# s0phia-/tetris

Hardware: AMD Instinct MI355X
Metric: env-steps/sec (higher is better)
Workload: dtype u32; 1 GPU; 1048576 envs/GPU x 1 GPU, 10x20 board, pieces=default, uniform random valid actions, in-kernel auto-reset, device bag seed 0; envs_per_gpu=1048576, observation_output=True, env_steps_per_launch=1, steps_per_graph_replay=1, streams_per_gpu=1, board=10x20, pieces=default, backend=single, device=cuda

## Files before the change

### tetris_amd/csrc/tetris_core.hpp

```cpp
#pragma once
#include <stdint.h>

#if defined(__HIPCC__)
#include <hip/hip_runtime.h>
#define TET_HD __host__ __device__ __forceinline__
#else
#define TET_HD inline
#endif

#ifndef TET_ABLATE
#define TET_ABLATE 0
#endif
#ifndef TET_BAG_SMALL_PATH
#define TET_BAG_SMALL_PATH 1
#endif
#ifndef TET_RESCUE_SKIP
#define TET_RESCUE_SKIP 1
#endif

#ifndef TET_FENCE_EVERY
#define TET_FENCE_EVERY 2
#endif
#ifndef TET_FENCE_MASK
#define TET_FENCE_MASK 1
#endif
#if defined(__HIP_DEVICE_COMPILE__)
#define TET_SCHED_FENCE() __builtin_amdgcn_sched_barrier(0)
#define TET_PIN(x) asm volatile("" : "+v"(x))
#else
#define TET_SCHED_FENCE() ((void)0)
#define TET_PIN(x) ((void)0)
#endif

#if defined(__HIP_DEVICE_COMPILE__)
#define TET_WAVE_ANY(x) (__ballot((x)) != 0ull)
#else
#define TET_WAVE_ANY(x) (x)
#endif

#if defined(__HIP_DEVICE_COMPILE__)
#define TET_SCRATCH_OR(ptr, v) ((void)__hip_atomic_fetch_or((ptr), (v), __ATOMIC_RELAXED, __HIP_MEMORY_SCOPE_WORKGROUP))
#else
#define TET_SCRATCH_OR(ptr, v) (*(ptr) |= (v))
#endif

#if defined(__HIP_DEVICE_COMPILE__)
#define TET_FMUL(a, b) __fmul_rn((a), (b))
#define TET_FADD(a, b) __fadd_rn((a), (b))
#else
#define TET_FMUL(a, b) ((float)((volatile float)(a) * (b)))
#define TET_FADD(a, b) ((float)((volatile float)(a) + (b)))
#endif

namespace tet {

constexpr int kMaxPieces = 12;
constexpr int kMaxCols = 12;
constexpr int kNumCatalogue = 9;

struct Orient {
  int w, H, b[4], n[4];
  bool exists;
};

TET_HD Orient unpack_orient(uint32_t d) {
  Orient o;
  o.w = d & 7;
  o.H = (d >> 3) & 7;
#pragma unroll
  for (int j = 0; j < 4; ++j) {
    o.b[j] = (d >> (6 + 5 * j)) & 3;
    o.n[j] = (d >> (8 + 5 * j)) & 7;
  }
  o.exists = (d >> 31) != 0;
  return o;
}

#ifndef TET_NO_PACK
#define TET_NO_PACK 0
#endif
TET_HD constexpr bool board_packed(int word_bytes, int num_rows) { return !TET_NO_PACK && num_rows + 4 <= 6 * word_bytes; }
TET_HD constexpr int n_planes(int C, bool packed) { return packed ? (C / 4) * 3 + ((C % 4) * 3 + 3) / 4 : C; }
constexpr int kTileEnvs = 64;
TET_HD constexpr int64_t plane_index(int64_t i, int p, int NP) { return ((i >> 6) * NP + p) * kTileEnvs + (i & 63); }
TET_HD constexpr int64_t board_words(int64_t B, int NP) { return ((B + kTileEnvs - 1) / kTileEnvs) * NP * kTileEnvs; }

template <typename W, int C, bool PACK>
TET_HD void unpack_board(const W (&w)[n_planes(C, PACK)], W (&col)[C]) {
  if (!PACK) {
#pragma unroll
    for (int c = 0; c < C; ++c) col[c] = w[c < n_planes(C, PACK) ? c : 0];
    return;
  }
  constexpr int Wb = 8 * (int)sizeof(W), F = Wb * 3 / 4, P = n_planes(C, PACK);
  const W M = (W)(((W)1 << F) - 1);
#pragma unroll
  for (int g = 0; 4 * g < C; ++g) {
    const int b = 3 * g, c0 = 4 * g;
    const W w0 = w[b], w1 = w[b + 1 < P ? b + 1 : b], w2 = w[b + 2 < P ? b + 2 : b];
    col[c0] = (W)(w0 & M);
    if (c0 + 1 < C) col[c0 + 1] = (W)(((w0 >> F) | (w1 << (Wb - F))) & M);
    if (c0 + 2 < C) col[c0 + 2] = (W)(((w1 >> (2 * F - Wb)) | (w2 << (2 * Wb - 2 * F))) & M);
    if (c0 + 3 < C) col[c0 + 3] = (W)(w2 >> (3 * F - 2 * Wb));
  }
}

template <typename W, int C, bool PACK>
TET_HD void pack_board(const W (&col)[C], W (&w)[n_planes(C, PACK)]) {
  if (!PACK) {
#pragma unroll
    for (int c = 0; c < n_planes(C, PACK); ++c) w[c] = col[c < C ? c : 0];
    return;
  }
  constexpr int Wb = 8 * (int)sizeof(W), F = Wb * 3 / 4, P = n_planes(C, PACK);
#pragma unroll
  for (int g = 0; 4 * g < C; ++g) {
    const int b = 3 * g, c0 = 4 * g;
    const W x0 = col[c0], x1 = c0 + 1 < C ? col[c0 + 1 < C ? c0 + 1 : c0] : (W)0;
    const W x2 = c0 + 2 < C ? col[c0 + 2 < C ? c0 + 2 : c0] : (W)0, x3 = c0 + 3 < C ? col[c0 + 3 < C ? c0 + 3 : c0] : (W)0;
    w[b] = (W)(x0 | (x1 << F));
    if (b + 1 < P) w[b + 1 < P ? b + 1 : b] = (W)((x1 >> (Wb - F)) | (x2 << (2 * F - Wb)));
    if (b + 2 < P) w[b + 2 < P ? b + 2 : b] = (W)((x2 >> (2 * Wb - 2 * F)) | (x3 << (3 * F - 2 * Wb)));
  }
}

template <typename W, int C, bool PACK>
TET_HD void load_board(const W* planes, int64_t , int64_t i, W (&col)[C]) {
  constexpr int NP = n_planes(C, PACK);
  W w[NP];
  const W* rec = planes + plane_index(i, 0, NP);
#pragma unroll
  for (int p = 0; p < NP; ++p) w[p] = rec[p * kTileEnvs];
  unpack_board<W, C, PACK>(w, col);
}
template <typename W, int C, bool PACK>
TET_HD void store_board(W* planes, int64_t , int64_t i, const W (&col)[C]) {
  constexpr int NP = n_planes(C, PACK);
  W w[NP];
  pack_board<W, C, PACK>(col, w);
  W* rec = planes + plane_index(i, 0, NP);
#pragma unroll
  for (int p = 0; p < NP; ++p) rec[p * kTileEnvs] = w[p];
}

template <typename W>
TET_HD W load_column_rt(const W* planes, int64_t , int64_t i, int c, int C, bool packed) {
  const int NP = n_planes(C, packed);
  if (!packed) return planes[plane_index(i, c, NP)];
  constexpr int Wb = 8 * (int)sizeof(W), F = Wb * 3 / 4;
  const W M = (W)(((W)1 << F) - 1);
  const int b = 3 * (c >> 2), k = c & 3;
  const W lo = planes[plane_index(i, b + (k == 0 ? 0 : k - 1), NP)];
  if (k == 0) return (W)(lo & M);
  if (k == 3) return (W)(lo >> (3 * F - 2 * Wb));
  const W hi = planes[plane_index(i, b + k, NP)];
  return k == 1 ? (W)(((lo >> F) | (hi << (Wb - F))) & M) : (W)(((lo >> (2 * F - Wb)) | (hi << (2 * Wb - 2 * F))) & M);
}
template <typename W>
TET_HD void store_columns_rt(W* planes, int64_t , int64_t i, const W* col, int C, bool packed) {
  if (!packed) {
    for (int c = 0; c < C; ++c) planes[plane_index(i, c, C)] = col[c];
    return;
  }
  constexpr int Wb = 8 * (int)sizeof(W), F = Wb * 3 / 4;
  const int P = n_planes(C, true);
  for (int p = 0; p < P; ++p) {
    const int c0 = 4 * (p / 3), q = p % 3;
    const W a = c0 + q < C ? col[c0 + q] : (W)0, b = c0 + q + 1 < C ? col[c0 + q + 1] : (W)0;
    const W v = q == 0 ? (W)(a | (b << F))
                       : (q == 1 ? (W)((a >> (Wb - F)) | (b << (2 * F - Wb))) : (W)((a >> (2 * Wb - 2 * F)) | (b << (3 * F - 2 * Wb))));
    planes[plane_index(i, p, P)] = v;
  }
}

constexpr uint64_t kMaskBits = (1ull << 48) - 1;
constexpr int kFieldStride = 12;
TET_HD constexpr int mask_bit(int k, int c) { return kFieldStride * k + c; }
TET_HD uint64_t meta_pack(uint64_t mask, int piece, uint32_t bag) {
  return (mask & kMaskBits) | ((uint64_t)(piece & 15) << 48) | ((uint64_t)(bag & 0xFFF) << 52);
}
TET_HD uint64_t meta_mask(uint64_t m) { return m & kMaskBits; }
TET_HD int meta_piece(uint64_t m) { return (int)((m >> 48) & 15); }
TET_HD uint32_t meta_bag(uint64_t m) { return (uint32_t)(m >> 52); }

TET_HD int popc(uint32_t x) { return __builtin_popcount(x); }
TET_HD int popc(uint64_t x) { return __builtin_popcountll(x); }
TET_HD int bitlen(uint32_t x) { return 31 - __builtin_clz((x << 1) | 1u); }
TET_HD int bitlen(uint64_t x) { return 63 - __builtin_clzll((x << 1) | 1ull); }
TET_HD uint32_t umin(uint32_t a, uint32_t b) { return a < b ? a : b; }
TET_HD int nlz_above(uint32_t x) { return __builtin_clz((x << 1) | 1u); }
TET_HD int nlz_above(uint64_t x) { return __builtin_clzll((x << 1) | 1ull); }
template <typename W>
TET_HD W lowmask(int n) { return (W)(((W)1 << n) - 1); }

TET_HD uint32_t sad_u8(uint32_t a, uint32_t b, uint32_t acc) {
#if defined(__HIP_DEVICE_COMPILE__)
  return __builtin_amdgcn_sad_u8(a, b, acc);
#else
  for (int k = 0; k < 4; ++k) {
    const int d = (int)((a >> (8 * k)) & 255u) - (int)((b >> (8 * k)) & 255u);
    acc += (uint32_t)(d < 0 ? -d : d);
  }
  return acc;
#endif
}

TET_HD uint32_t mix32(uint32_t x) {
  x ^= x >> 16;
  x *= 0x7feb352dU;
  x ^= x >> 15;
  x *= 0x846ca68bU;
  x ^= x >> 16;
  return x;
}
TET_HD uint32_t hash_key(uint64_t seed, uint64_t counter) {
  uint32_t k = mix32((uint32_t)seed ^ 0x9E3779B9U);
  k = mix32(k ^ (uint32_t)(seed >> 32));
  k = mix32(k ^ (uint32_t)counter);
  k = mix32(k ^ (uint32_t)(counter >> 32));
  return k;
}
TET_HD uint32_t hash_env(uint32_t key, uint32_t env) {
  uint32_t h = (key ^ env) * 0x9E3779B1U;
  h ^= h >> 16;
  h *= 0x85EBCA6BU;
  h ^= h >> 13;
  return h;
}
TET_HD int scale16(uint32_t r16, int n) { return (int)((r16 * (uint32_t)n) >> 16); }

TET_HD int select_bit32(uint32_t v, int k) {
  int pos = 0;
  int c = popc(v & 0xFFFFu);
  if (k >= c) { k -= c; pos += 16; v >>= 16; }
  c = popc(v & 0xFFu);
  if (k >= c) { k -= c; pos += 8; v >>= 8; }
  c = popc(v & 0xFu);
  if (k >= c) { k -= c; pos += 4; v >>= 4; }
  c = popc(v & 0x3u);
  if (k >= c) { k -= c; pos += 2; v >>= 2; }
  c = (int)(v & 1u);
  if (k >= c) { pos += 1; }
  return pos;
}
TET_HD int bag_draw(uint32_t& bag, int n_pieces, uint32_t r16) {
  if (bag == 0) bag = (1u << n_pieces) - 1u;
  const int k = scale16(r16, popc(bag));
  uint32_t v = bag;
  int pos = 0;
  int c = popc(v & 0xFFu);
  if (k >= c) { pos = 8; v >>= 8; }
  int kk = k >= c ? k - c : k;
  c = popc(v & 0xFu);
  if (kk >= c) { kk -= c; pos += 4; v >>= 4; }
  c = popc(v & 0x3u);
  if (kk >= c) { kk -= c; pos += 2; v >>= 2; }
  c = (int)(v & 1u);
  if (kk >= c) pos += 1;
  bag &= ~(1u << pos);
  return pos;
}

TET_HD int bag_draw_lut(uint32_t& bag, int n_pieces, uint32_t r16, const uint8_t* sel_nib) {
  if (bag == 0) bag = (1u << n_pieces) - 1u;
#if TET_BAG_SMALL_PATH
  if (n_pieces <= 4) {
    const int k4 = scale16(r16, popc(bag));
    const int pos4 = (int)sel_nib[bag * 4u + (uint32_t)k4];
    bag &= ~(1u << pos4);
    return pos4;
  }
#endif
  int k = scale16(r16, popc(bag));
  const int c0 = popc(bag & 0xFu), c1 = c0 + popc(bag & 0xF0u);
  const int grp = (k >= c0) + (k >= c1);
  k -= grp == 0 ? 0 : (grp == 1 ? c0 : c1);
  const uint32_t nib = (bag >> (4 * grp)) & 15u;
  const int pos = 4 * grp + (int)sel_nib[nib * 4u + (uint32_t)k];
  bag &= ~(1u << pos);
  return pos;
}

struct alignas(16) OrientEntry {
  uint32_t sh[4];
  uint32_t rj0[2];
  uint32_t rj1[2];
  uint32_t vert4;
  uint32_t set_w4;
  uint32_t desc;
  uint32_t pad_;
};
static_assert(sizeof(OrientEntry) == 48, "table staging and LDS reads assume 48-byte entries");

struct alignas(16) StampRow {
  uint32_t shape4;
  uint32_t bias4;
  uint32_t H;
  uint32_t pad_;
};
constexpr uint32_t kNoColumn = 64;
static_assert(sizeof(StampRow) == 16, "one ds_read_b128");

struct SetTable {
  OrientEntry orient[kMaxPieces][4];
  uint64_t fullmask[kMaxPieces];
  StampRow stamp[kMaxPieces][4];
};

TET_HD const OrientEntry* piece_entries(const SetTable& tab, int np) {
  uint32_t off = (uint32_t)np * (uint32_t)sizeof(tab.orient[0]);
  TET_PIN(off);
  return reinterpret_cast<const OrientEntry*>(reinterpret_cast<const char*>(&tab.orient[0][0]) + off);
}

template <int CR>
struct LutLayout {
  static constexpr int kHoleEntries = 1 << (CR + 1), kWellsEntries = 1 << CR;
  static constexpr int kHoleA = 0, kHoleU = kHoleEntries, kWellsS = 2 * kHoleEntries;
  static constexpr int kWellsLead = kWellsS + kWellsEntries, kWellsTrail = kWellsLead + kWellsEntries;
  static constexpr int kSelPair = kWellsTrail + kWellsEntries, kSelNib = kSelPair + 256 * 8;
  static constexpr int kByteTablesEnd = kSelNib + 16 * 4;
  static constexpr int kPackHole = kByteTablesEnd, kPackWells = kPackHole + 2 * kHoleEntries;
  static constexpr int kBytes = CR == 10 ? kPackWells + 4 * kWellsEntries : kByteTablesEnd;
};
template <typename W, int C, int NCH, int CR, bool PACKW = false>
TET_HD constexpr bool features_packed() { return sizeof(W) == 4 && C <= 10 && NCH == 2 && CR == 10 && !PACKW; }
constexpr int kFeatureLutBytes = LutLayout<12>::kBytes;
constexpr int kFeatureLut10Bytes = LutLayout<10>::kBytes;
struct AfterLut {
  static constexpr int kHoleA = LutLayout<12>::kHoleA, kHoleU = LutLayout<12>::kHoleU;
  static constexpr int kWellsPack = 2 * LutLayout<12>::kHoleEntries;
  static constexpr int kSelPair = kWellsPack + 4 * LutLayout<12>::kWellsEntries, kSelNib = kSelPair + 256 * 8;
  static constexpr int kBytes = kSelNib + 16 * 4;
};
constexpr int kAfterLutBytes = AfterLut::kBytes;

TET_HD uint32_t spread2(uint32_t x) {
  x = (x | (x << 8)) & 0x00FF00FFu;
  x = (x | (x << 4)) & 0x0F0F0F0Fu;
  x = (x | (x << 2)) & 0x33333333u;
  x = (x | (x << 1)) & 0x55555555u;
  return x;
}

template <int C>
TET_HD uint32_t mask_field(uint64_t mask, int k) { return (uint32_t)(mask >> (kFieldStride * k)) & ((1u << C) - 1u); }

template <int C>
TET_HD void slot_of_action_lut(uint64_t mask, int k, const uint8_t* sel_pair, int& kk, int& c) {
  static_assert(C <= 12, "three 4-column groups per 12-bit field");
  constexpr uint32_t kLoopBits = (1u << (2 * kFieldStride)) - 1u;
  const uint32_t w0 = (uint32_t)mask & kLoopBits, w1 = (uint32_t)(mask >> (2 * kFieldStride)) & kLoopBits;
  const int n0 = popc(w0);
  const bool second = k >= n0;
  const uint32_t w = second ? w1 : w0;
  int kr = second ? k - n0 : k;
  constexpr uint32_t kG0 = 0xFu | (0xFu << kFieldStride);
  const int c0 = popc(w & kG0), c1 = c0 + popc(w & (kG0 << 4));
  const int grp = (C > 4 ? (kr >= c0) : 0) + (C > 8 ? (kr >= c1) : 0);
  kr -= grp == 0 ? 0 : (grp == 1 ? c0 : c1);
  const uint32_t t = w >> (4 * grp);
  const uint32_t idx = (t & 15u) | (((t >> kFieldStride) & 15u) << 4);
  const uint32_t r = sel_pair[idx * 8u + (uint32_t)kr];
  c = 4 * grp + (int)(r & 3u);
  kk = (second ? 2 : 0) + (int)(r >> 2);
}
template <int C>
TET_HD void slot_of_action(uint64_t mask, int k, int& kk, int& c) {
  const uint32_t f0 = mask_field<C>(mask, 0), f1 = mask_field<C>(mask, 1);
  const uint32_t f2 = mask_field<C>(mask, 2), f3 = mask_field<C>(mask, 3);
  const int n0 = popc(f0) + popc(f1);
  const bool second = k >= n0;
  const uint32_t z = spread2(second ? f2 : f0) | (spread2(second ? f3 : f1) << 1);
  const int pos = select_bit32(z, second ? k - n0 : k);
  c = pos >> 1;
  kk = (second ? 2 : 0) + (pos & 1);
}
template <int C>
TET_HD int row_of_slot(uint64_t mask, int kk, int c) {
  const int L = kk >> 1;
  const uint32_t fa = mask_field<C>(mask, 2 * L), fb = mask_field<C>(mask, 2 * L + 1);
  const uint32_t below = (1u << c) - 1u;
  int row = popc(fa & below) + popc(fb & below) + ((kk & 1) ? (int)((fa >> c) & 1u) : 0);
  if (L) row += popc(mask_field<C>(mask, 0)) + popc(mask_field<C>(mask, 1));
  return row;
}

template <typename W, int C>
TET_HD void heights_of(const W (&col)[C], int (&h)[C]) {
#pragma unroll
  for (int c = 0; c < C; ++c) h[c] = bitlen(col[c]);
}

template <typename W, int C>
TET_HD int stamp_static(const W (&col)[C], const int (&h)[C], int c, const Orient& o, W (&nb)[C],
                        W (&pbits)[4]) {
  int a = -64;
#pragma unroll
  for (int j = 0; j < 4; ++j)
    if (c + j < C) {
      int v = (j < o.w) ? h[c + j] - o.b[j] : -64;
      a = v > a ? v : a;
    }
  if (a < 0) a = 0;
#pragma unroll
  for (int i = 0; i < C; ++i) nb[i] = col[i];
#pragma unroll
  for (int j = 0; j < 4; ++j) {
    int nj = (j < o.w) ? o.n[j] : 0;
    pbits[j] = (W)(lowmask<W>(nj) << (a + o.b[j]));
    if (c + j < C) nb[c + j] |= pbits[j];
  }
  return a;
}

template <typename W, int C>
TET_HD int clear_lines(W (&col)[C], const W (&pbits)[4], int a, int* eroded_cells) {
  W F = (W)((W)~(W)0 << a);
#pragma unroll
  for (int i = 0; i < C; ++i) F &= col[i];
  int k = popc(F);
  int er = 0;
  if (F != 0) {
#pragma unroll
    for (int j = 0; j < 4; ++j) er += popc((W)(F & pbits[j]));
    while (F != 0) {
      int p = bitlen(F) - 1;
      W low = lowmask<W>(p);
#pragma unroll
      for (int i = 0; i < C; ++i) col[i] = (W)((col[i] & low) | ((col[i] >> (p + 1)) << p));
      F = (W)(F & low);
    }
  }
  *eroded_cells = er;
  return k;
}

template <typename W, int NCH = 0, int CR = 12>
TET_HD void col_own(W x, int hi, int R, const uint8_t* lut, W& ho, int& nh, int& f1, int& f7) {
  ho = (W)(~x & lowmask<W>(hi));
  nh = popc(ho);
  const uint8_t* lut_a = lut + LutLayout<CR>::kHoleA;
  const uint8_t* lut_u = lut + LutLayout<CR>::kHoleU;
  int d7 = 0, u = 0;
  if (!(TET_ABLATE & 16)) {
#pragma unroll
    for (int k = 0; CR * k < (int)(8 * sizeof(W)) - 1; ++k) {
      if (NCH > 0 ? k < NCH : (k < 2 || CR * k < R + 4)) {
        const uint32_t up = (uint32_t)(x >> (CR * k));
        const uint32_t idx = (NCH > 0 && k == NCH - 1) ? up : (up & (uint32_t)(LutLayout<CR>::kHoleEntries - 1));
        const int uk = lut_u[idx];
        u += uk;
        d7 += lut_a[idx];
        const bool more = NCH > 0 ? k + 1 < NCH : (CR * (k + 1) < R + 4);
        if (CR * (k + 1) < (int)(8 * sizeof(W)) && more) d7 += uk * popc((W)(x >> (CR * (k + 1))));
      }
    }
  }
  f1 = 2 * u;
  f7 = d7;
}

template <typename W>
TET_HD int col_rowtrans(W x, W L, int hi, int hL, int nh_left) {
  const int dl = hL - hi;
  return popc((W)((x ^ L) & lowmask<W>(hi))) + (dl > 0 ? dl : 0) - ((hi == 0) ? nh_left : 0);
}

template <typename W, int NCH = 0, int CR = 12>
TET_HD int col_wells(W x, W L, W Rr, int hi, int R, bool left_wall, bool right_wall, const uint8_t* lut) {
  W w = (W)(~x & L & Rr);
  if (left_wall || right_wall) w = (W)(w & lowmask<W>(hi > R ? hi : R));
  const uint8_t* lut_s = lut + LutLayout<CR>::kWellsS;
  const uint8_t* lut_lead = lut + LutLayout<CR>::kWellsLead;
  const uint8_t* lut_trail = lut + LutLayout<CR>::kWellsTrail;
  int total = 0, carry = 0;
#pragma unroll
  for (int k = 0; CR * k < (int)(8 * sizeof(W)) - 1; ++k) {
    if (NCH > 0 ? k < NCH : (k < 2 || CR * k < R + 4)) {
      const uint32_t up = (uint32_t)(w >> (CR * k));
      const uint32_t idx = (NCH > 0 && k == NCH - 1) ? up : (up & (uint32_t)(LutLayout<CR>::kWellsEntries - 1));
      const bool last = NCH > 0 && k == NCH - 1;
      total += lut_s[idx];
      if (k == 0) {
        if (!last) carry = lut_trail[idx];
      } else {
        const int lead = lut_lead[idx];
        total += carry * lead;
        if (!last) {
          const int trail = lut_trail[idx];
          carry = (lead == CR) ? carry + CR : trail;
        }
      }
    }
  }
  return (TET_ABLATE & 32) ? 0 : total;
}

template <typename W, int NCH = 0>
TET_HD int col_wells_packed(W x, W L, W Rr, int hi, int R, bool left_wall, bool right_wall, const uint32_t* pack) {
  constexpr int CR = 12;
  W w = (W)(~x & L & Rr);
  if (left_wall || right_wall) w = (W)(w & lowmask<W>(hi > R ? hi : R));
  uint32_t total = 0, carry = 0;
#pragma unroll
  for (int k = 0; CR * k < (int)(8 * sizeof(W)) - 1; ++k) {
    if (NCH > 0 ? k < NCH : (k < 2 || CR * k < R + 4)) {
      const uint32_t up = (uint32_t)(w >> (CR * k));
      const bool last = NCH > 0 && k == NCH - 1;
      const uint32_t e = pack[last ? up : (up & 4095u)];
      total += e & 0xFFFFu;
      const uint32_t lead = e >> 24, trail = (e >> 16) & 255u;
      if (k == 0) {
        if (!last) carry = trail;
      } else {
        total += carry * lead;
        if (!last) carry = (lead == (uint32_t)CR) ? carry + (uint32_t)CR : trail;
      }
    }
  }
  return (int)total;
}

template <int C>
TET_HD void board_features_u32_2x10(const uint32_t (&col)[C], int R, const uint8_t* lut, int& rows_with_holes,
                                    int& col_trans, int& holes, int& wells, int& row_trans, int& hole_depth) {
  static_assert(C <= 12, "three words of packed heights");
  typedef LutLayout<10> LL;
  constexpr int CR = 10;
  const uint16_t* hole_pack = reinterpret_cast<const uint16_t*>(lut + LL::kPackHole);
  const uint32_t* wells_pack = reinterpret_cast<const uint32_t*>(lut + LL::kPackWells);
  const uint32_t wall = lowmask<uint32_t>(R + 4);
  const uint32_t nwall = (uint32_t)(31 - R);
  uint32_t n[C];
  uint32_t P[3] = {0u, 0u, 0u};
#pragma unroll
  for (int c = 0; c < C; ++c) {
    n[c] = (uint32_t)__builtin_clz((col[c] << 1) | 1u);
    P[c >> 2] |= n[c] << (8 * (c & 3));
  }
  uint32_t sad = (C % 4 == 0) ? n[C - 1] : 0u;
#pragma unroll
  for (int q = 0; q < (C + 3) / 4; ++q) {
    const uint32_t Q = (P[q] << 8) | (q == 0 ? nwall : (P[q > 0 ? q - 1 : 0] >> 24));
    sad = sad_u8(P[q], Q, sad);
  }
  uint32_t hole_rows = 0;
  uint32_t hsum = 0, wsum = 0;
  uint32_t f2 = 0, f4 = 0, f7 = 0;
  uint32_t f5 = (uint32_t)(R - popc(col[C - 1])) + ((sad - nwall) >> 1);
  uint32_t f5neg = 0;
  uint32_t nh_left = 0;
#pragma unroll
  for (int i = 0; i < C; ++i) {
    const uint32_t x = col[i];
    const uint32_t L = (i == 0) ? wall : col[i > 0 ? i - 1 : 0];
    const uint32_t Rr = (i == C - 1) ? wall : col[i + 1 < C ? i + 1 : i];
    const uint32_t lm = 0x7FFFFFFFu >> n[i];
    const uint32_t ho = ~x & lm;
    const uint32_t nh = (uint32_t)popc(ho);
    f2 += nh;
    hole_rows |= ho;
    f5 += (uint32_t)popc((x ^ L) & lm);
    f5neg += (x == 0u) ? nh_left : 0u;
    nh_left = nh;
    if (!(TET_ABLATE & 16)) {
      const uint32_t i0 = x & (uint32_t)(LL::kHoleEntries - 1), i1 = x >> CR;
      const uint32_t e0 = hole_pack[i0];
      hsum += e0 + hole_pack[i1];
      f7 += (e0 & 255u) * (uint32_t)popc(i1);
    }
    if (!(TET_ABLATE & 32)) {
      uint32_t w = ~x & L & Rr;
      if (i == 0 || i == C - 1) w &= 0x7FFFFFFFu >> (n[i] < nwall ? n[i] : nwall);
      const uint32_t i0 = w & (uint32_t)(LL::kWellsEntries - 1), i1 = w >> CR;
      const uint32_t e0 = wells_pack[i0], e1 = wells_pack[i1];
      wsum += e0 + e1;
      f4 += (e0 & 255u) * ((e1 >> 8) & 255u);
    }
    if (TET_FENCE_EVERY > 0 && i % TET_FENCE_EVERY == TET_FENCE_EVERY - 1 && i + 1 < C) {
      TET_PIN(hsum);
      TET_PIN(wsum);
      TET_PIN(f2);
      TET_PIN(f4);
      TET_PIN(f5);
      TET_PIN(f7);
      TET_SCHED_FENCE();
    }
  }
  rows_with_holes = popc(hole_rows);
  col_trans = C + 2 * (int)(hsum & 255u);
  holes = (int)f2;
  wells = (int)(f4 + (wsum >> 16));
  row_trans = (int)(f5 - f5neg);
  hole_depth = (int)(f7 + (hsum >> 8));
}

template <typename W, int C, int NCH = 0, int CR = 12, bool PACKW = false>
TET_HD void board_features(const W (&col)[C], const int (&h)[C], int R, const uint8_t* hole_lut,
                           int& rows_with_holes, int& col_trans, int& holes, int& wells, int& row_trans,
                           int& hole_depth) {
  if constexpr (features_packed<W, C, NCH, CR, PACKW>()) {
    board_features_u32_2x10<C>(col, R, hole_lut, rows_with_holes, col_trans, holes, wells, row_trans, hole_depth);
    return;
  }
  const W wall = lowmask<W>(R + 4);
  W hole_rows = 0;
  int f1 = C;
  int f2 = 0, f4 = 0, f7 = 0;
  int f5 = R - popc(col[C - 1]);
// ... 575 lines not shown
```

### tetris_amd/csrc/tetris_kernels.hip

```cpp
#include <hip/hip_runtime.h>
#include <stdlib.h>
#include <string.h>

#include "../../include/tetris_hip.h"
#include "tetris_entry.hpp"

namespace {

using tet::SetTable;
using tet::StepCfg;

constexpr int kBlock = 256;

#ifndef TET_STEP_WAVES
#define TET_STEP_WAVES 0
#endif
template <typename W, int CR = 12>
constexpr int step_waves() { return TET_STEP_WAVES ? TET_STEP_WAVES : (sizeof(W) == 4 ? 5 : (CR == 10 ? 4 : 3)); }

#ifndef TET_STEP_BLOCK
#define TET_STEP_BLOCK 0
#endif
template <typename W>
constexpr int step_block() { return TET_STEP_BLOCK ? TET_STEP_BLOCK : (sizeof(W) == 4 ? 512 : 256); }

#ifndef TET_STAMPS
#define TET_STAMPS 0
#endif
#if TET_STAMPS
constexpr int kStampWgs = 16384, kStampWords = 20;
__device__ uint64_t g_stamps[kStampWgs * kStampWords];
#define TET_STAMP(slot) do { if (threadIdx.x == 0 && blockIdx.x < kStampWgs) g_stamps[blockIdx.x * kStampWords + (slot)] = __builtin_amdgcn_s_memrealtime(); } while (0)
#else
#define TET_STAMP(slot) ((void)0)
#endif


static_assert(tet::kAfterLutBytes % 16 == 0, "staged as uint4");
template <int CR>
__device__ __forceinline__ const uint4* feature_lut_src() {
  return CR == 10 ? reinterpret_cast<const uint4*>(&kFeatureLut10) : reinterpret_cast<const uint4*>(&kFeatureLut);
}
__device__ __forceinline__ void stage_after_lut(uint8_t* lds) {
  const uint4* src = reinterpret_cast<const uint4*>(&kAfterLut);
  uint4* dst = reinterpret_cast<uint4*>(lds);
  for (int t = threadIdx.x; t < tet::kAfterLutBytes / 16; t += blockDim.x) dst[t] = src[t];
}

template <typename W, int C, int BLK, int CR, bool AFTER = false>
struct alignas(16) StepLds {
  SetTable tab;
  alignas(16) uint8_t lut[AFTER ? tet::kAfterLutBytes
                                : (tet::features_packed<W, C, 2, CR>() ? tet::LutLayout<CR>::kBytes : tet::LutLayout<CR>::kByteTablesEnd)];
  W lane_cols[tet::scratch_cols<W, C, 2, CR, AFTER>()][BLK];
};

template <typename W, int C, int NCH, int CR>
constexpr int lut_stage_begin() { return tet::features_packed<W, C, NCH, CR>() ? tet::LutLayout<CR>::kSelPair / 16 : 0; }
template <typename W, int C, int NCH, int CR>
constexpr int lut_stage_end() {
  return (tet::features_packed<W, C, NCH, CR>() ? tet::LutLayout<CR>::kBytes : tet::LutLayout<CR>::kByteTablesEnd) / 16;
}
static_assert(tet::LutLayout<10>::kSelPair % 16 == 0 && tet::LutLayout<10>::kByteTablesEnd % 16 == 0 && tet::LutLayout<10>::kBytes % 16 == 0, "staged as uint4");

template <typename W, int C, int NCH, int CR>
__device__ __forceinline__ void stage_hole_lut(uint8_t* lds) {
  const uint4* src = feature_lut_src<CR>();
  uint4* dst = reinterpret_cast<uint4*>(lds);
  for (int t = lut_stage_begin<W, C, NCH, CR>() + (int)threadIdx.x; t < lut_stage_end<W, C, NCH, CR>(); t += blockDim.x) dst[t] = src[t];
}

__device__ __forceinline__ void stage_table(SetTable& lds, const SetTable& arg) {
  const uint32_t* src = reinterpret_cast<const uint32_t*>(&arg);
  uint32_t* dst = reinterpret_cast<uint32_t*>(&lds);
  for (int t = threadIdx.x; t < (int)(sizeof(SetTable) / 4); t += blockDim.x) dst[t] = src[t];
  __syncthreads();
}

__device__ __forceinline__ unsigned wave_sum(int value_bits, int v) {
  unsigned total = 0;
  for (int b = 0; b < value_bits; ++b) {
    unsigned long long m = __ballot((v >> b) & 1);
    total += (unsigned)__popcll(m) << b;
  }
  return total;
}
__device__ __forceinline__ unsigned wave_count(bool cond) { return (unsigned)__popcll(__ballot(cond)); }

template <typename T>
__device__ __forceinline__ T ld_off(const T* base, uint32_t byte_off) {
  return *reinterpret_cast<const T*>(reinterpret_cast<const char*>(base) + byte_off);
}
template <typename T>
__device__ __forceinline__ void st_off(T* base, uint32_t byte_off, T v) {
  *reinterpret_cast<T*>(reinterpret_cast<char*>(base) + byte_off) = v;
}

template <typename W, int NP>
__device__ __forceinline__ uint32_t record_off(uint32_t i) {
  return ((i >> 6) * (uint32_t)(NP * 64) + (i & 63u)) * (uint32_t)sizeof(W);
}
template <typename W, int C, bool PACK>
__device__ __forceinline__ void store_planes(const StepParams& p, uint32_t i, const W (&col)[C]) {
  constexpr int NP = tet::n_planes(C, PACK);
  W w[NP];
  tet::pack_board<W, C, PACK>(col, w);
  const uint32_t off = record_off<W, NP>(i);
#pragma unroll
  for (int q = 0; q < NP; ++q) st_off(static_cast<W*>(p.cols), off + (uint32_t)(q * 64 * sizeof(W)), w[q]);
}

template <typename W, int C>
struct StepInputs {
  W col[C];
  uint64_t meta;
  int action;
  int draw, draw_reset, cursor;
  bool exhausted;
  uint4 status;
};

template <typename W, int C, bool PACK>
__device__ __forceinline__ void load_inputs(const StepParams& p, uint32_t i, StepInputs<W, C>& in) {
  const uint32_t ii = i < p.B ? i : 0;
  constexpr int NP = tet::n_planes(C, PACK);
  W w[NP];
  const uint32_t off = record_off<W, NP>(ii);
#pragma unroll
  for (int q = 0; q < NP; ++q) w[q] = ld_off(static_cast<const W*>(p.cols), off + (uint32_t)(q * 64 * sizeof(W)));
  tet::unpack_board<W, C, PACK>(w, in.col);
  in.meta = ld_off(p.meta, ii * 8u);
  in.action = p.action ? ld_off(p.action, ii * 4u) : -1;
  tet::stream_read(p.stream, p.cursor, p.stream_len, p.B, ii, p.cfg, in.draw, in.draw_reset, in.cursor, in.exhausted);
  in.status = make_uint4(0, 0, 0, 0);
  if (p.status) in.status = ld_off(reinterpret_cast<const uint4*>(p.status), (i >> 6) * 16u);
}

template <typename W, int C, int NCH, int CR, int BLK = step_block<W>()>
__global__ __launch_bounds__(BLK, (step_waves<W, CR>())) void step_kernel(const StepParams p) {
  constexpr int kBlock = BLK;
  __shared__ StepLds<W, C, kBlock, CR> lds;
  SetTable& tab = lds.tab;
  uint8_t* const hole_lut = lds.lut;
  auto& lane_cols = lds.lane_cols;
  static_assert(sizeof(lds.lane_cols) / sizeof(lds.lane_cols[0]) >= (tet::scratch_padded<W, C, NCH, CR, false>() ? C + 3 : C), "the unclamped stamp needs its three columns");
  const uint32_t i = blockIdx.x * kBlock + threadIdx.x;
  const bool live = i < p.B;
  constexpr bool PACK = NCH != 0 && !TET_NO_PACK;
  TET_STAMP(0);
  StepInputs<W, C> in;
  load_inputs<W, C, PACK>(p, i, in);
  {
    constexpr int kLutVec0 = lut_stage_begin<W, C, NCH, CR>();
    constexpr int kLutVecs = lut_stage_end<W, C, NCH, CR>() - kLutVec0, kLutPerLane = (kLutVecs + kBlock - 1) / kBlock;
    const uint4* lsrc = feature_lut_src<CR>() + kLutVec0;
    uint4 lv[kLutPerLane];
#pragma unroll
    for (int q = 0; q < kLutPerLane; ++q) {
      const int t = (int)threadIdx.x + q * kBlock;
      lv[q] = lsrc[kLutVecs % kBlock == 0 || t < kLutVecs ? t : kLutVecs - 1];
    }
    constexpr int kTabWords = (int)(sizeof(SetTable) / 4), kTabPerLane = (kTabWords + kBlock - 1) / kBlock;
    const uint32_t* tsrc = reinterpret_cast<const uint32_t*>(&p.tab);
    uint32_t tw[kTabPerLane];
#pragma unroll
    for (int q = 0; q < kTabPerLane; ++q)
      tw[q] = (int)threadIdx.x + q * kBlock < kTabWords ? tsrc[threadIdx.x + q * kBlock] : 0u;
#pragma unroll
    for (int q = 0; q < kLutPerLane; ++q)
      if (!(TET_ABLATE & 128) && (kLutVecs % kBlock == 0 || (int)threadIdx.x + q * kBlock < kLutVecs))
        reinterpret_cast<uint4*>(hole_lut)[kLutVec0 + threadIdx.x + q * kBlock] = lv[q];
#pragma unroll
    for (int q = 0; q < kTabPerLane; ++q)
      if ((int)threadIdx.x + q * kBlock < kTabWords) reinterpret_cast<uint32_t*>(&tab)[threadIdx.x + q * kBlock] = tw[q];
    __syncthreads();
  }
  TET_STAMP(1);
  StepCfg cfg = p.cfg;
  if (p.step_counter) {
    const uint64_t c = *p.step_counter;
    const uint64_t idx = (((uint64_t)__builtin_amdgcn_readfirstlane((uint32_t)(c >> 32)) << 32) |
                          __builtin_amdgcn_readfirstlane((uint32_t)c)) + p.step_rel;
    cfg.key_step = tet::hash_key(p.seed, idx * 4u + 0u);
    cfg.key_policy = tet::hash_key(p.seed, idx * 4u + 3u);
  }
  bool invalid = false, done = false, done_flag = false;
  int lines = 0;
  if (live) {
    tet::StepOut out;
    tet::env_step<W, C, NCH, CR, false, tet::scratch_padded<W, C, NCH, CR>()>(in.col, in.meta, in.exhausted ? -1 : in.action, p.action == nullptr && !in.exhausted,
                             tab, hole_lut, &lane_cols[0][threadIdx.x], kBlock, cfg, p.env_offset + i, in.draw,
                             in.draw_reset, out);
    invalid = out.invalid != 0;
    TET_STAMP(2);
    if (p.obs) {
      float4* o4 = reinterpret_cast<float4*>(p.obs);
      st_off(o4, i * 32u, make_float4(out.obs[0], out.obs[1], out.obs[2], out.obs[3]));
      st_off(o4, i * 32u + 16u, make_float4(out.obs[4], out.obs[5], out.obs[6], out.obs[7]));
    }
    if (!invalid) {
      store_planes<W, C, PACK>(p, i, in.col);
      st_off(p.meta, i * 8u, in.meta);
      done = out.done != 0;
      lines = out.lines;
      if (p.stream) p.cursor[i] = in.cursor + 1 + ((out.done && cfg.auto_reset) ? 1 : 0);
    }
    done_flag = out.done != 0;
    st_off(p.reward, i * 4u, (int32_t)out.reward);
    st_off(p.done, i, (uint8_t)out.done);
    st_off(p.lines, i, (uint8_t)out.lines);
    st_off(p.n_valid, i, (uint8_t)out.n_valid);
    if (p.piece_next) st_off(p.piece_next, i, (uint8_t)out.piece);
    if (p.action_out) st_off(p.action_out, i * 4u, (int32_t)out.action);
  }
  if (!(TET_ABLATE & 8192) && (p.status || p.done_bits)) {
    const unsigned long long done_mask = __ballot(done_flag);
    const unsigned n_inv = wave_count(invalid);
    const unsigned n_done = wave_count(done);
    const unsigned n_lines = wave_sum(3, lines);
    const unsigned n_steps = wave_count(live && !invalid);
    if ((threadIdx.x & 63) == 0) {
      uint4 v = in.status;
      v.x += n_inv;
      v.y += n_done;
      v.z += n_lines;
      v.w += n_steps;
      if (p.status) st_off(reinterpret_cast<uint4*>(p.status), (i >> 6) * 16u, v);
      if (p.status_snapshot) st_off(reinterpret_cast<uint4*>(p.status_snapshot), (i >> 6) * 16u, v);
      if (p.done_bits && (i & ~63u) < p.B) st_off(p.done_bits, (i >> 6) * 8u, done_mask);
    }
  }
#if TET_STAMPS
  __syncthreads();
  if (threadIdx.x == 0 && blockIdx.x < kStampWgs) {
    asm volatile("s_waitcnt vmcnt(0)" ::: "memory");
    g_stamps[blockIdx.x * kStampWords + 3] = __builtin_amdgcn_s_memrealtime();
    g_stamps[blockIdx.x * kStampWords + 4] = __builtin_amdgcn_s_getreg(63492);
    g_stamps[blockIdx.x * kStampWords + 5] = __builtin_amdgcn_s_getreg(63508);
  }
#endif
}

#ifndef TET_AFTER_WAVES
#define TET_AFTER_WAVES 2
#endif
#ifndef TET_GREEDY_WAVES
#define TET_GREEDY_WAVES 3
#endif
#ifndef TET_STEP_GREEDY_WAVES
#define TET_STEP_GREEDY_WAVES 4
#endif
#ifndef TET_AFTER_WAVES64
#define TET_AFTER_WAVES64 2
#endif
template <typename W, int C>
constexpr int after_waves(int want) {
  return sizeof(W) == 4 ? want : (want > TET_AFTER_WAVES64 ? TET_AFTER_WAVES64 : want);
}

template <typename W, int C, int NCH, int POLICY, int CR>
__global__ __launch_bounds__(step_block<W>(), (POLICY == 0 ? step_waves<W, CR>() : after_waves<W, C>(TET_STEP_GREEDY_WAVES))) void step_many_kernel(const StepManyParams q) {
  static_assert(POLICY == 0 || CR == 12, "the greedy policy evaluates terminal afterstates too: 12-row chunks");
  constexpr int kBlock = step_block<W>();
  const StepParams& p = q.one;
  constexpr bool AFTER = POLICY == 1;
  __shared__ StepLds<W, C, kBlock, CR, AFTER> lds;
  SetTable& tab = lds.tab;
  uint8_t* const hole_lut = lds.lut;
  auto& lane_cols = lds.lane_cols;
  static_assert(sizeof(lds.lane_cols) / sizeof(lds.lane_cols[0]) >= (tet::scratch_padded<W, C, NCH, CR, AFTER>() ? C + 3 : C), "the unclamped stamp needs its three columns");
  const uint32_t i = blockIdx.x * kBlock + threadIdx.x;
  const bool live = i < p.B;
  constexpr bool PACK = NCH != 0 && !TET_NO_PACK;
  StepInputs<W, C> in;
  load_inputs<W, C, PACK>(p, i, in);
  if (AFTER) stage_after_lut(hole_lut);
  else stage_hole_lut<W, C, NCH, CR>(hole_lut);
  stage_table(tab, p.tab);
  unsigned n_inv = 0, n_done = 0, n_lines = 0, n_steps = 0;
  StepCfg cfg = p.cfg;
#pragma unroll 1
  for (int k = 0; k < q.n_steps; ++k) {
    cfg.key_step = tet::hash_key(q.seed, (q.step_idx0 + (uint64_t)k) * 4u + 0u);
    cfg.key_policy = tet::hash_key(q.seed, (q.step_idx0 + (uint64_t)k) * 4u + 3u);
    bool invalid = false, done = false;
    int lines = 0;
    if (live) {
      int action = -1;
      bool use_policy = true;
      if (POLICY == 1) {
        float best = 0.f;
        int best_row = -1;
        tet::afterstates_env<W, C, NCH>(in.col, in.meta, tab, hole_lut, cfg.R, [&](bool has, int, int, float (&f)[8], int, int row, bool is_valid) {
          if (!has) return;
          if (is_valid) {
            const float v = tet::fitness_of(f, q.w);
            if (best_row < 0 || v > best || (v == best && row < best_row)) {
              best = v;
              best_row = row;
            }
          }
        });
        action = best_row;
        use_policy = false;
      }
      tet::StepOut out;
      tet::env_step<W, C, NCH, CR, AFTER, tet::scratch_padded<W, C, NCH, CR, AFTER>()>(in.col, in.meta, action, use_policy, tab, hole_lut, &lane_cols[0][threadIdx.x],
                                          kBlock, cfg, p.env_offset + i, -1, -1, out);
      invalid = out.invalid != 0;
      const uint32_t e = (uint32_t)k * p.B + i;
      if (p.obs) {
        float4* o4 = reinterpret_cast<float4*>(p.obs);
        st_off(o4, e * 32u, make_float4(out.obs[0], out.obs[1], out.obs[2], out.obs[3]));
        st_off(o4, e * 32u + 16u, make_float4(out.obs[4], out.obs[5], out.obs[6], out.obs[7]));
      }
      if (!invalid) {
        done = out.done != 0;
        lines = out.lines;
      }
      st_off(p.reward, e * 4u, (int32_t)out.reward);
      st_off(p.done, e, (uint8_t)out.done);
      st_off(p.lines, e, (uint8_t)out.lines);
      st_off(p.n_valid, e, (uint8_t)out.n_valid);
      if (p.piece_next) st_off(p.piece_next, e, (uint8_t)out.piece);
      if (p.action_out) st_off(p.action_out, e * 4u, (int32_t)out.action);
    }
    n_inv += wave_count(invalid);
    n_done += wave_count(done);
    n_lines += wave_sum(3, lines);
    n_steps += wave_count(live && !invalid);
  }
  if (live) {
    store_planes<W, C, PACK>(p, i, in.col);
    st_off(p.meta, i * 8u, in.meta);
  }
  if (p.status && (threadIdx.x & 63) == 0) {
    uint4 v = in.status;
    v.x += n_inv;
    v.y += n_done;
    v.z += n_lines;
    v.w += n_steps;
    st_off(reinterpret_cast<uint4*>(p.status), (i >> 6) * 16u, v);
  }
}

template <typename W, int C, bool PACK>
__global__ __launch_bounds__(kBlock) void reset_kernel(const ResetParams p) {
  __shared__ SetTable tab;
  stage_table(tab, p.tab);
  const int64_t i = (int64_t)blockIdx.x * kBlock + threadIdx.x;
  const bool mine = i < p.B && !(p.reset_mask && !p.reset_mask[i]);
  const int cur = (mine && p.stream) ? p.cursor[i] : 0;
  const bool exhausted = mine && p.stream && tet::stream_reset_exhausted(cur, p.stream_len);
  if (p.status) {
    const unsigned n_bad = (unsigned)__popcll(__ballot(exhausted));
    if ((threadIdx.x & 63) == 0 && n_bad) p.status[(i >> 6) * 4 + TETRIS_STATUS_INVALID] += n_bad;
  }
  if (!mine || exhausted) return;
  tet::reset_env<W, C, PACK>(static_cast<W*>(p.cols), p.meta, p.B, i, tab, p.init_bag, p.n_pieces, p.key, p.env_offset, p.stream,
                             p.cursor, cur, p.piece_out, p.n_valid_out);
}

template <typename W, int C, bool PACK>
__global__ __launch_bounds__(kBlock) void refresh_kernel(const RefreshParams p) {
  __shared__ SetTable tab;
  stage_table(tab, p.tab);
  const int64_t i = (int64_t)blockIdx.x * kBlock + threadIdx.x;
  if (i >= p.B) return;
  tet::refresh_env<W, C, PACK>(static_cast<const W*>(p.cols), p.meta, p.n_valid_out, p.B, i, tab, p.R);
}



__device__ __forceinline__ uint32_t swap_neighbour(uint32_t v) {
  return (uint32_t)__builtin_amdgcn_mov_dpp((int)v, 0xB1, 0xF, 0xF, true);
}
__device__ __forceinline__ void store_row_paired(float* base, bool has, uint32_t at4, const float (&f)[8]) {
  const bool odd = threadIdx.x & 1u;
  const uint32_t at_mine = has ? at4 : ~0u;
  const uint32_t at_other = swap_neighbour(at_mine);
  float r[4];
#pragma unroll
  for (int q = 0; q < 4; ++q)
    r[q] = __uint_as_float(swap_neighbour(__float_as_uint(odd ? f[q] : f[q + 4])));
  const uint32_t d_even = odd ? at_other : at_mine, d_odd = odd ? at_mine : at_other;
  const float4 v_even = odd ? make_float4(r[0], r[1], r[2], r[3]) : make_float4(f[0], f[1], f[2], f[3]);
  const float4 v_odd = odd ? make_float4(f[4], f[5], f[6], f[7]) : make_float4(r[0], r[1], r[2], r[3]);
  float4* out = reinterpret_cast<float4*>(base);
  const uint32_t part = odd ? 1u : 0u;
  if (d_even != ~0u) out[(size_t)d_even + part] = v_even;
  if (d_odd != ~0u) out[(size_t)d_odd + part] = v_odd;
}

template <typename W, int C, int NCH>
__global__ __launch_bounds__(kBlock, (after_waves<W, C>(TET_AFTER_WAVES))) void afterstates_kernel(const AfterParams p) {
  __shared__ SetTable tab;
  __shared__ __attribute__((aligned(16))) uint8_t hole_lut[tet::kAfterLutBytes];
  stage_after_lut(hole_lut);
  stage_table(tab, p.tab);
  const int64_t i0 = (int64_t)blockIdx.x * kBlock + threadIdx.x;
  const bool live = i0 < p.B;
  const int64_t i = live ? i0 : p.B - 1;
  const W* cols = static_cast<const W*>(p.cols);
  W col[C];
  tet::load_board<W, C, (NCH != 0 && !TET_NO_PACK)>(cols, p.B, i, col);
  const uint64_t meta = p.meta[i];
  const int piece = tet::meta_piece(meta);
  const uint64_t full = tab.fullmask[piece];
  const uint64_t valid = tet::meta_mask(meta) & full;
  const uint32_t es4 = (uint32_t)(p.env_stride / 4), rs4 = (uint32_t)(p.row_stride / 4);
  const uint32_t env4 = (uint32_t)i * es4;
  const int nv = tet::popc(valid), na = tet::popc(full);
  float sink = 0.f;
  tet::afterstates_env<W, C, NCH>(col, meta, tab, hole_lut, p.R, [&](bool has, int sk, int sc, float (&f)[8], int row_all, int row_valid, bool is_valid) {
    has = has && live;
    if (TET_ABLATE & 64) {
      if (has) sink += f[0] + f[1] + f[2] + f[3] + f[4] + f[5] + f[6] + f[7] + (float)(sk + sc);
      return;
    }
    if (p.has_direct_by) {
#pragma unroll
      for (int q = 0; q < 8; ++q) f[q] *= p.direct_by[q];
    }
    if (p.feats_all) store_row_paired(p.feats_all, has, env4 + (uint32_t)row_all * rs4, f);
    store_row_paired(p.feats, has && is_valid, env4 + (uint32_t)row_valid * rs4, f);
  });
  if (TET_ABLATE & 64) {
    if (live) p.feats[i * p.env_stride] = sink;
    return;
  }
  {
    const bool odd = threadIdx.x & 1u;
    const uint32_t part = odd ? 1u : 0u;
    const uint32_t env4_o = swap_neighbour(env4);
    const int nv_o = (int)swap_neighbour((uint32_t)(live ? nv : 0x7FFFFFFF)), na_o = (int)swap_neighbour((uint32_t)(live ? na : 0x7FFFFFFF));
    const int nv_m = live ? nv : 0x7FFFFFFF, na_m = live ? na : 0x7FFFFFFF;
    const uint32_t base_e = odd ? env4_o : env4, base_o = odd ? env4 : env4_o;
    const int nv_e = odd ? nv_o : nv_m, nv_od = odd ? nv_m : nv_o, na_e = odd ? na_o : na_m, na_od = odd ? na_m : na_o;
    const float4 z4 = make_float4(0.f, 0.f, 0.f, 0.f);
    float4* out = reinterpret_cast<float4*>(p.feats);
    float4* out_all = reinterpret_cast<float4*>(p.feats_all);
    for (int k = 0; k < p.a_max; ++k) {
      const uint32_t r4 = (uint32_t)k * rs4 + part;
      if (k >= nv_e) out[(size_t)base_e + r4] = z4;
      if (k >= nv_od) out[(size_t)base_o + r4] = z4;
      if (out_all) {
        if (k >= na_e) out_all[(size_t)base_e + r4] = z4;
        if (k >= na_od) out_all[(size_t)base_o + r4] = z4;
      }
    }
  }
  if (live) {
    p.n_valid[i] = (uint8_t)nv;
    if (p.n_all) p.n_all[i] = (uint8_t)na;
  }
}


template <typename W, int C, int NCH>
__global__ __launch_bounds__(kBlock, (after_waves<W, C>(TET_GREEDY_WAVES))) void greedy_kernel(const GreedyParams p) {
  __shared__ SetTable tab;
  __shared__ __attribute__((aligned(16))) uint8_t hole_lut[tet::kAfterLutBytes];
  stage_after_lut(hole_lut);
  stage_table(tab, p.tab);
  const int64_t i = (int64_t)blockIdx.x * kBlock + threadIdx.x;
  if (i >= p.B) return;
  const W* cols = static_cast<const W*>(p.cols);
  W col[C];
  tet::load_board<W, C, (NCH != 0 && !TET_NO_PACK)>(cols, p.B, i, col);
  const uint64_t meta = p.meta[i];
  const int piece = tet::meta_piece(meta);
  const uint64_t full = tab.fullmask[piece];
  const uint64_t valid = tet::meta_mask(meta) & full;
  float* fall = p.fitness_all ? p.fitness_all + i * (int64_t)p.a_max : nullptr;
  tet::GreedyPick pick;
  tet::afterstates_env<W, C, NCH>(col, meta, tab, hole_lut, p.R, [&](bool has, int, int, float (&f)[8], int row_all, int row, bool is_valid) {
    if (!has) return;
    const float v = tet::fitness_of(f, p.w);
    if (fall && !(TET_ABLATE & 2048)) fall[row_all] = v;
    if (is_valid) pick.offer(v, row);
  });
  if (fall)
    for (int k = tet::popc(full); k < p.a_max; ++k) fall[k] = 0.f;
  p.best_action[i] = pick.best_row;
  if (p.best_value) p.best_value[i] = pick.best;
}

constexpr int kRolloutBlock = 512;
template <typename W, int C, int NCH>
__global__ __launch_bounds__(kRolloutBlock, (after_waves<W, C>(TET_STEP_GREEDY_WAVES))) void rollouts_kernel(const RolloutParams p) {
  constexpr int kBlock = kRolloutBlock;
  __shared__ StepLds<W, C, kBlock, 12, true> lds;
  SetTable& tab = lds.tab;
  uint8_t* const hole_lut = lds.lut;
  auto& lane_cols = lds.lane_cols;
  stage_after_lut(hole_lut);
  stage_table(tab, p.tab);
  const int64_t id = (int64_t)blockIdx.x * kBlock + threadIdx.x;
  if (id >= p.B * p.a_max) return;
  const int64_t i = id / p.a_max;
  const int a0 = (int)(id - i * p.a_max);
  const W* cols = static_cast<const W*>(p.cols);
// ... 320 lines not shown
```

Baseline: 37.72 billion env-steps/s.

## Swap observation halves across lanes for contiguous stores; stage only used table rows

Observation output is now written after a permlane32 swap, so each float4 store instruction covers a contiguous span of rows rather than alternating halves of 32-byte records, which should coalesce global writes better. The per-block SetTable staging now loads and writes only the words belonging to the active number of pieces, cutting global loads and LDS writes. The swap requires every lane to take part, so obs is zero-initialised for dead lanes and rows are bounds-checked against B; it relies on the gfx950 permlane32_swap builtin.

```diff
diff --git a/tetris_amd/csrc/tetris_core.hpp b/tetris_amd/csrc/tetris_core.hpp
--- a/tetris_amd/csrc/tetris_core.hpp
+++ b/tetris_amd/csrc/tetris_core.hpp
@@ -1,4 +1,5 @@
 #pragma once
+#include <stddef.h>
 #include <stdint.h>
 
 #if defined(__HIPCC__)
@@ -306,6 +307,21 @@
   uint64_t fullmask[kMaxPieces];
   StampRow stamp[kMaxPieces][4];
 };
+
+constexpr int kOrientRowWords = (int)(4 * sizeof(OrientEntry) / 4), kStampRowWords = (int)(4 * sizeof(StampRow) / 4);
+constexpr int kFullmaskWord0 = kMaxPieces * kOrientRowWords, kStampWord0 = kFullmaskWord0 + 2 * kMaxPieces;
+constexpr int kSetTableWords = (int)(sizeof(SetTable) / 4);
+static_assert(offsetof(SetTable, fullmask) == 4 * kFullmaskWord0 && offsetof(SetTable, stamp) == 4 * kStampWord0 &&
+              kSetTableWords == kStampWord0 + kMaxPieces * kStampRowWords, "set_table_word_staged walks the three arrays");
+template <int LO = 0, int HI = kSetTableWords>
+TET_HD bool set_table_word_staged(int word, int n_pieces) {
+  bool used = false;
+  if (LO < kFullmaskWord0) used = word < n_pieces * kOrientRowWords;
+  if (HI > kFullmaskWord0 && LO < kStampWord0) used = used || (uint32_t)(word - kFullmaskWord0) < (uint32_t)(2 * n_pieces);
+  if (HI > kStampWord0) used = used || (uint32_t)(word - kStampWord0) < (uint32_t)(n_pieces * kStampRowWords);
+  return used;
+}
+constexpr int set_table_staged_bytes(int n_pieces) { return 4 * n_pieces * (kOrientRowWords + 2 + kStampRowWords); }
 
 TET_HD const OrientEntry* piece_entries(const SetTable& tab, int np) {
   uint32_t off = (uint32_t)np * (uint32_t)sizeof(tab.orient[0]);
diff --git a/tetris_amd/csrc/tetris_kernels.hip b/tetris_amd/csrc/tetris_kernels.hip
--- a/tetris_amd/csrc/tetris_kernels.hip
+++ b/tetris_amd/csrc/tetris_kernels.hip
@@ -1,6 +1,8 @@
 #include <hip/hip_runtime.h>
 #include <stdlib.h>
 #include <string.h>
+
+#include <utility>
 
 #include "../../include/tetris_hip.h"
 #include "tetris_entry.hpp"
@@ -70,6 +72,11 @@
   for (int t = lut_stage_begin<W, C, NCH, CR>() + (int)threadIdx.x; t < lut_stage_end<W, C, NCH, CR>(); t += blockDim.x) dst[t] = src[t];
 }
 
+template <int BLK, int... Q>
+__device__ __forceinline__ void table_words_staged(int n_pieces, bool (&tu)[sizeof...(Q)], std::integer_sequence<int, Q...>) {
+  ((tu[Q] = tet::set_table_word_staged<Q * BLK, (Q + 1) * BLK>((int)threadIdx.x + Q * BLK, n_pieces)), ...);
+}
+
 __device__ __forceinline__ void stage_table(SetTable& lds, const SetTable& arg) {
   const uint32_t* src = reinterpret_cast<const uint32_t*>(&arg);
   uint32_t* dst = reinterpret_cast<uint32_t*>(&lds);
@@ -94,6 +101,21 @@
 template <typename T>
 __device__ __forceinline__ void st_off(T* base, uint32_t byte_off, T v) {
   *reinterpret_cast<T*>(reinterpret_cast<char*>(base) + byte_off) = v;
+}
+
+__device__ __forceinline__ void store_obs_rows(float* obs, uint32_t i, uint32_t B, const float (&f)[8]) {
+  uint32_t a[4], b[4];
+#pragma unroll
+  for (int q = 0; q < 4; ++q) {
+    auto r = __builtin_amdgcn_permlane32_swap(__float_as_uint(f[q]), __float_as_uint(f[q + 4]), false, false);
+    a[q] = r[0];
+    b[q] = r[1];
+  }
+  const uint32_t lane = i & 63u, row = (i & ~63u) + (lane & 31u);
+  const uint32_t off = row * 32u + (lane >> 5) * 16u;
+  float4* o4 = reinterpret_cast<float4*>(obs);
+  if (row < B) st_off(o4, off, make_float4(__uint_as_float(a[0]), __uint_as_float(a[1]), __uint_as_float(a[2]), __uint_as_float(a[3])));
+  if (row + 32u < B) st_off(o4, off + 1024u, make_float4(__uint_as_float(b[0]), __uint_as_float(b[1]), __uint_as_float(b[2]), __uint_as_float(b[3])));
 }
 
 template <typename W, int NP>
@@ -160,19 +182,20 @@
       const int t = (int)threadIdx.x + q * kBlock;
       lv[q] = lsrc[kLutVecs % kBlock == 0 || t < kLutVecs ? t : kLutVecs - 1];
     }
-    constexpr int kTabWords = (int)(sizeof(SetTable) / 4), kTabPerLane = (kTabWords + kBlock - 1) / kBlock;
+    constexpr int kTabWords = tet::kSetTableWords, kTabPerLane = (kTabWords + kBlock - 1) / kBlock;
     const uint32_t* tsrc = reinterpret_cast<const uint32_t*>(&p.tab);
     uint32_t tw[kTabPerLane];
-#pragma unroll
-    for (int q = 0; q < kTabPerLane; ++q)
-      tw[q] = (int)threadIdx.x + q * kBlock < kTabWords ? tsrc[threadIdx.x + q * kBlock] : 0u;
+    bool tu[kTabPerLane];
+    table_words_staged<kBlock>(p.cfg.n_pieces, tu, std::make_integer_sequence<int, kTabPerLane>());
+#pragma unroll
+    for (int q = 0; q < kTabPerLane; ++q) tw[q] = tu[q] ? tsrc[threadIdx.x + q * kBlock] : 0u;
 #pragma unroll
     for (int q = 0; q < kLutPerLane; ++q)
       if (!(TET_ABLATE & 128) && (kLutVecs % kBlock == 0 || (int)threadIdx.x + q * kBlock < kLutVecs))
         reinterpret_cast<uint4*>(hole_lut)[kLutVec0 + threadIdx.x + q * kBlock] = lv[q];
 #pragma unroll
     for (int q = 0; q < kTabPerLane; ++q)
-      if ((int)threadIdx.x + q * kBlock < kTabWords) reinterpret_cast<uint32_t*>(&tab)[threadIdx.x + q * kBlock] = tw[q];
+      if (tu[q]) reinterpret_cast<uint32_t*>(&tab)[threadIdx.x + q * kBlock] = tw[q];
     __syncthreads();
   }
   TET_STAMP(1);
@@ -186,18 +209,18 @@
   }
   bool invalid = false, done = false, done_flag = false;
   int lines = 0;
+  tet::StepOut out;
+#pragma unroll
+  for (int q = 0; q < 8; ++q) out.obs[q] = 0.f;
   if (live) {
-    tet::StepOut out;
     tet::env_step<W, C, NCH, CR, false, tet::scratch_padded<W, C, NCH, CR>()>(in.col, in.meta, in.exhausted ? -1 : in.action, p.action == nullptr && !in.exhausted,
                              tab, hole_lut, &lane_cols[0][threadIdx.x], kBlock, cfg, p.env_offset + i, in.draw,
                              in.draw_reset, out);
+    TET_STAMP(2);
+  }
+  if (p.obs) store_obs_rows(p.obs, i, p.B, out.obs);
+  if (live) {
     invalid = out.invalid != 0;
-    TET_STAMP(2);
-    if (p.obs) {
-      float4* o4 = reinterpret_cast<float4*>(p.obs);
-      st_off(o4, i * 32u, make_float4(out.obs[0], out.obs[1], out.obs[2], out.obs[3]));
-      st_off(o4, i * 32u + 16u, make_float4(out.obs[4], out.obs[5], out.obs[6], out.obs[7]));
-    }
     if (!invalid) {
       store_planes<W, C, PACK>(p, i, in.col);
       st_off(p.meta, i * 8u, in.meta);
```

Result: no change. 37.71 billion env-steps/s (-0.0%).
